# zfountas/deep-active-inference-mc

Measured on AMD Instinct MI355X. Metric: EFE rollouts/sec (64x64 dSprites, 10 MC-samples, depth 5), higher is better.
Workload: dtype f32; 1 GPU; calculate_G_repeated: 128 rows (32 roots x 4 actions) x depth 5 x 10 MC samples per GPU (BASELINE configs[1]) + action posterior; rows_per_gpu=128, samples=10, depth=5, parallelism=episodes sharded x1, weights replicated

## Files before the change

### deep-active-inference-mc_amd/csrc/decoder.hip

```cpp
#include <utility>
#include "mfma_pipe.h"

namespace efe {

template <class F, int... I> __device__ __forceinline__ void static_for_(F&& f, std::integer_sequence<int, I...>) { (f(std::integral_constant<int, I>{}), ...); }
template <int N, class F> __device__ __forceinline__ void static_for(F&& f) { static_for_(f, std::make_integer_sequence<int, N>{}); }

__host__ __device__ constexpr int w3_nch(int G) { return G == 4 ? 5 : 4; }
__host__ __device__ constexpr int w3_prod(int G, int c) {
    return G < 4 ? 5 * ((G >> 1) + 2 * (c >> 1)) + (G & 1) + 2 * (c & 1)
         : G == 4 ? (c < 2 ? 5 * (1 + 2 * c) + 4 : c < 4 ? 20 + 1 + 2 * (c - 2) : 24)
                  : (c < 2 ? 5 * (2 * c) + 4 : 20 + 2 * (c - 2));
}
__host__ __device__ constexpr bool w3_direct(int pp) { return f22_o1(pp / 5) < 0 && f22_o1(pp % 5) < 0; }
__host__ __device__ constexpr int w3_view(int pp) { return 3 * f22_view(pp / 5) + f22_view(pp % 5); }
__host__ __device__ constexpr int w3_mat(int pp) { return 4 * f22_wt(pp / 5) + f22_wt(pp % 5); }
__host__ __device__ constexpr bool w3_hits(int pp, int o) {
    const int r = o >> 2, c = o & 3, pr = pp / 5, pc = pp % 5;
    return (r == f22_o0(pr) || r == f22_o1(pr)) && (c == f22_o0(pc) || c == f22_o1(pc));
}
__host__ __device__ constexpr bool w3_seen(int G, int c, int o) {
    for (int g = 0; g < G; ++g)
        for (int k = 0; k < w3_nch(g); ++k) if (w3_hits(w3_prod(g, k), o)) return true;
    if (!w3_direct(w3_prod(G, c)))
        for (int k = 0; k < w3_nch(G); ++k)
            if ((w3_direct(w3_prod(G, k)) || k < c) && w3_hits(w3_prod(G, k), o)) return true;
    return false;
}
__host__ __device__ constexpr bool w3_uses_view(int G, int vi) {
    for (int k = 0; k < w3_nch(G); ++k) if (w3_view(w3_prod(G, k)) == vi) return true;
    return false;
}
__host__ __device__ constexpr bool f22_in(int a, int r) { return a == 0 ? r <= 1 : (a == 1 ? r == 1 : r >= 1); }
__host__ __device__ constexpr bool w3_reads(int G, int r, int c) {
    for (int vi = 0; vi < 9; ++vi) if (w3_uses_view(G, vi) && f22_in(vi / 3, r) && f22_in(vi % 3, c)) return true;
    return false;
}

constexpr int DA_PS = 17;
constexpr int DA_BIAS = 273 * DA_PS;

__host__ __device__ constexpr int wino_i0(int a) { return a == 0 ? 0 : (a == 2 ? 2 : 1); }
__host__ __device__ constexpr int wino_i1(int a) { return a == 0 ? 2 : (a == 1 ? 2 : (a == 2 ? 1 : 3)); }
__host__ __device__ constexpr float wino_s1(int a) { return a == 1 ? 1.0f : -1.0f; }
__host__ __device__ constexpr float wino_at(int r, int a) { return r == 0 ? (a < 3 ? 1.0f : 0.0f) : (a == 0 ? 0.0f : (a == 1 ? 1.0f : -1.0f)); }

template <int NR, int R0, class Pix>
__device__ __forceinline__ void wino_l1(f32x16 (&out)[NR][2], const float4* __restrict__ U, const float4* sm, const int h,
                                        const int mt_, Pix pix) {
    constexpr int PD = 4;
    const unsigned ln = (threadIdx.x & 63u) * 16u;
    const __amdgpu_buffer_rsrc_t ur = wrsrc(U);
    int mt = mt_; asm volatile("" : "+s"(mt));
    constexpr int a_lo = NR == 2 ? 0 : R0, a_hi = NR == 2 ? 4 : R0 + 3;
    auto ufrag = [&](int a, int b, int kc) { return wfrag(ur, ln, (size_t)(((4 * a + b) * 2 + mt) * 8 + kc) * 64); };
    auto bases = [&](int a, int b, int (&pb)[4]) {
        const int i0 = wino_i0(a), i1 = wino_i1(a), j0 = wino_i0(b), j1 = wino_i1(b);
        pb[0] = pix(i0, j0); pb[1] = pix(i0, j1); pb[2] = pix(i1, j0); pb[3] = pix(i1, j1);
    };
    float4 aq[PD], raw[4];
    int pb[4];
#pragma unroll
    for (int p = 0; p < PD; ++p) aq[p] = ufrag(a_lo, 0, p);
    bases(a_lo, 0, pb);
#pragma unroll
    for (int q = 0; q < 4; ++q) raw[q] = sm[pb[q] + h];
    f32x16 xacc;
    const f32x16 zero = {};
    auto otrans = [&](int a, int b, const f32x16& m, auto mask) {
        constexpr int MASK = decltype(mask)::value;
#pragma unroll
        for (int r = 0; r < NR; ++r) {
            if (!((MASK >> r) & 1)) continue;
            const float car = wino_at(R0 + r, a);
#pragma unroll
            for (int c = 0; c < 2; ++c) {
                const float cbc = wino_at(c, b);
                if (cbc == 0.0f) continue;
                const float cf = car * cbc;
#pragma unroll
                for (int e = 0; e < 16; ++e) out[r][c][e] = __builtin_fmaf(cf, m[e], out[r][c][e]);
            }
        }
    };
    auto xi_row = [&](int a, auto mask) {
        const float s1 = wino_s1(a);
        const int an = a + 1 < a_hi ? a + 1 : a;
#pragma unroll
        for (int b = 0; b < 4; ++b) {
            const float t1 = wino_s1(b);
#pragma unroll
            for (int kc = 0; kc < 8; ++kc) {
                const float4 av = aq[kc % PD];
                aq[kc % PD] = (b * 8 + kc + PD < 32) ? ufrag(a, (b * 8 + kc + PD) >> 3, (kc + PD) & 7) : ufrag(an, 0, (kc + PD) & 7);
                float4 v;
                {
                    const float4 c0 = make_float4(__builtin_fmaf(s1, raw[2].x, raw[0].x), __builtin_fmaf(s1, raw[2].y, raw[0].y),
                                                  __builtin_fmaf(s1, raw[2].z, raw[0].z), __builtin_fmaf(s1, raw[2].w, raw[0].w));
                    const float4 c1 = make_float4(__builtin_fmaf(s1, raw[3].x, raw[1].x), __builtin_fmaf(s1, raw[3].y, raw[1].y),
                                                  __builtin_fmaf(s1, raw[3].z, raw[1].z), __builtin_fmaf(s1, raw[3].w, raw[1].w));
                    v = make_float4(__builtin_fmaf(t1, c1.x, c0.x), __builtin_fmaf(t1, c1.y, c0.y), __builtin_fmaf(t1, c1.z, c0.z), __builtin_fmaf(t1, c1.w, c0.w));
                }
                if (kc < 7) {
#pragma unroll
                    for (int q = 0; q < 4; ++q) raw[q] = sm[pb[q] + 2 * (kc + 1) + h];
                } else {
                    if (b < 3) bases(a, b + 1, pb);
                    else bases(an, 0, pb);
#pragma unroll
                    for (int q = 0; q < 4; ++q) raw[q] = sm[pb[q] + h];
                }
                __builtin_amdgcn_sched_barrier(0);
                f32x16& x = xacc;
                x = __builtin_amdgcn_mfma_f32_32x32x2f32(av.x, v.x, kc == 0 ? zero : x, 0, 0, 0);
                x = __builtin_amdgcn_mfma_f32_32x32x2f32(av.y, v.y, x, 0, 0, 0);
                x = __builtin_amdgcn_mfma_f32_32x32x2f32(av.z, v.z, x, 0, 0, 0);
                x = __builtin_amdgcn_mfma_f32_32x32x2f32(av.w, v.w, x, 0, 0, 0);
            }
            otrans(a, b, xacc, mask);
        }
    };
    if constexpr (NR == 2) {
        xi_row(0, std::integral_constant<int, 1>{});
#pragma unroll 1
        for (int a = 1; a < 3; ++a) xi_row(a, std::integral_constant<int, 3>{});
        xi_row(3, std::integral_constant<int, 2>{});
    } else {
#pragma unroll 1
        for (int a = a_lo; a < a_hi; ++a) xi_row(a, std::integral_constant<int, 1>{});
    }
}
struct F22Nb { int xb, c2[3], r2; };
__device__ __forceinline__ f32x4 f22_wfrag(const __amdgpu_buffer_rsrc_t wr, const unsigned ln, int ct, int m, int kc) {
    return __builtin_bit_cast(f32x4, wfrag(wr, ln + (unsigned)kc * 1024u, (size_t)(m * 4 + ct) * 256));
}
constexpr int F22_PD = 2;
__device__ __forceinline__ void f22_l2_first(f32x4 (&aq)[F22_PD][5], const __amdgpu_buffer_rsrc_t wr, const int dn, const unsigned ln) {
    static_for<F22_PD>([&](auto p) {
        static_for<w3_nch(p >> 2)>([&](auto c) { aq[p][c] = f22_wfrag(wr, ln, dn, w3_mat(w3_prod(p >> 2, c)), p & 3); });
    });
}
__device__ __forceinline__ void f22_l2(f32x4 (&acc)[16], f32x4 (&aq)[F22_PD][5], const __amdgpu_buffer_rsrc_t wr, const int dn,
                                       const unsigned ln, const f32x4 bias4, const f32x4* smv, const F22Nb& nb) {
    constexpr int NST = 24;
    auto px = [&](int i, int jj, int kc) -> f32x4 {
        return smv[(jj == 2 ? nb.c2[i] : (i == 2 ? nb.r2 + jj * DA_PS : nb.xb + (16 * i + jj) * DA_PS)) + 4 * kc];
    };
    auto view = [&](const f32x4 (&x)[9], int vi) -> f32x4 {
        const int va = vi / 3, vb = vi % 3;
        auto cv = [&](int i) -> f32x4 { return vb == 0 ? x[3 * i] - x[3 * i + 1] : (vb == 1 ? x[3 * i + 1] : x[3 * i + 2] - x[3 * i + 1]); };
        return va == 0 ? cv(0) - cv(1) : (va == 1 ? cv(1) : cv(2) - cv(1));
    };
    const f32x4 zero4 = {};
    f32x4 tq[5], xr[9];
    static_for<9>([&](auto i) { if constexpr (w3_reads(0, i / 3, i % 3)) xr[i] = px(i / 3, i % 3, 0); });
    static_for<NST>([&](auto stc) {
        constexpr int ST = decltype(stc)::value, G = ST >> 2, KC = ST & 3, GN = (ST + 1) >> 2, KN = (ST + 1) & 3;
        constexpr int SP = (ST + F22_PD) % NST, GP = SP >> 2, KP = SP & 3;
        f32x4 vw[9], ac[5];
        static_for<9>([&](auto vi) { if constexpr (w3_uses_view(G, vi)) vw[vi] = view(xr, vi); });
#pragma unroll
        for (int c = 0; c < 5; ++c) ac[c] = aq[ST % F22_PD][c];
        static_for<w3_nch(GP)>([&](auto c) { aq[ST % F22_PD][c] = f22_wfrag(wr, ln, ST + F22_PD < NST ? 0 : dn, w3_mat(w3_prod(GP, c)), KP); });
        if constexpr (ST + 1 < NST)
            static_for<9>([&](auto i) { if constexpr (w3_reads(GN, i / 3, i % 3)) xr[i] = px(i / 3, i % 3, KN); });
        __builtin_amdgcn_sched_barrier(0);
#pragma unroll
        for (int e = 0; e < 4; ++e)
            static_for<w3_nch(G)>([&](auto c) {
                constexpr int PP = w3_prod(G, c);
                const float b = vw[w3_view(PP)][e], av = ac[c][e];
                if constexpr (w3_direct(PP)) {
                    constexpr int O = 4 * f22_o0(PP / 5) + f22_o0(PP % 5);
                    constexpr bool FIRST = KC == 0 && !w3_seen(G, c, O);
                    acc[O] = __builtin_amdgcn_mfma_f32_16x16x4f32(av, b, (FIRST && e == 0) ? bias4 : acc[O], 0, 0, 0);
                } else {
                    tq[c] = __builtin_amdgcn_mfma_f32_16x16x4f32(av, b, (KC == 0 && e == 0) ? zero4 : tq[c], 0, 0, 0);
                }
            });
        if constexpr (KC == 3)
            static_for<w3_nch(G)>([&](auto c) {
                constexpr int PP = w3_prod(G, c);
                if constexpr (!w3_direct(PP))
                    static_for<16>([&](auto o) {
                        if constexpr (w3_hits(PP, o)) {
                            if constexpr (w3_seen(G, c, o)) acc[o] = acc[o] + tq[c];
                            else acc[o] = bias4 + tq[c];
                        }
                    });
            });
    });
}
__device__ __forceinline__ void f22_l2_store(f32x4 (&acc)[16], const __amdgpu_buffer_rsrc_t yr, const unsigned yoff, const int ct, const bool on) {
#pragma unroll
    for (int orow = 0; orow < 4; ++orow)
#pragma unroll
        for (int c = 0; c < 2; ++c) {
            u32x4 lo, hi;
#pragma unroll
            for (int e = 0; e < 4; ++e) {
                const unsigned x0 = __builtin_bit_cast(unsigned, relu_bits(acc[4 * orow + c][e]));
                const unsigned x1 = __builtin_bit_cast(unsigned, relu_bits(acc[4 * orow + c + 2][e]));
                const auto sw = __builtin_amdgcn_permlane32_swap(x0, x1, false, false);
                lo[e] = sw[0]; hi[e] = sw[1];
            }
            const unsigned so = (unsigned)(((2 * (orow & 1) + c) * 4096 + 2 * ct * 512 + (orow >> 1) * 32) * 16);
            if (on) {
                __builtin_amdgcn_raw_buffer_store_b128(lo, yr, yoff, so, 0);
                __builtin_amdgcn_raw_buffer_store_b128(hi, yr, yoff, so + 512u * 16u, 0);
            }
        }
}

__global__ void __launch_bounds__(256, 2) k_dec_a(const DecAArgs a) {
    constexpr int NTHR = 256;
    constexpr int NPH = 2048 / NTHR;
    constexpr int NPE = 8;
    extern __shared__ __attribute__((aligned(16))) float4 sm[];
    const int tid = threadIdx.x;
    const int lane = tid & 63;
    const int w = __builtin_amdgcn_readfirstlane(tid >> 6);

    const float4* W1 = reinterpret_cast<const float4*>(a.w1);
    const float4* W2 = reinterpret_cast<const float4*>(a.w2);

    if ((int)blockIdx.x >= a.rows) return;
    int* const slot = reinterpret_cast<int*>(sm + DA_BIAS + 32);
    if (tid == 0) slot[0] = 2 * (int)gridDim.x + atomicAdd(a.queue, 1);
    int nimg = (int)blockIdx.x + (int)gridDim.x;
    f32x4 pf[2 * NPH];
    f32x4* smv = reinterpret_cast<f32x4*>(sm);
    {
        const f32x4* X = reinterpret_cast<const f32x4*>(a.x4) + (size_t)blockIdx.x * 4096;
#pragma unroll
        for (int it = 0; it < 2 * NPH; ++it) pf[it] = X[w * 1024 + it * 64 + lane];
    }
    for (int i = tid; i < 17 * DA_PS; i += NTHR) sm[256 * DA_PS + i] = make_float4(0.f, 0.f, 0.f, 0.f);
    if (tid < 16) sm[DA_BIAS + tid] = reinterpret_cast<const float4*>(a.b1)[tid];
    else if (tid < 32) sm[DA_BIAS + tid] = reinterpret_cast<const float4*>(a.b2)[tid - 16];

    for (int img = blockIdx.x; img < a.rows;) {
        int tl_ = tid; asm volatile("" : "+v"(tl_));
        const int j = tl_ & 31, h = (tl_ >> 5) & 1;
        const bool live = row_live(a.live, img);
        if (live) {
            const int sbase = (64 * w + ((tl_ >> 4) & 3)) * DA_PS + (tl_ & 15);
#pragma unroll
            for (int it = 0; it < 2 * NPH; ++it) smv[sbase + it * 4 * DA_PS] = pf[it];
        }
        __syncthreads();
        const int nnimg = slot[0];
        int ticket = 0;
        if (tid == 0) ticket = 2 * (int)gridDim.x + atomicAdd(a.queue, 1);
        const int l1mt = w >> 1, l1n = 32 * (w & 1) + j;
        const int l1y = 2 * (l1n >> 3) - 1, l1x = 2 * (l1n & 7) - 1;
        if (live) {
            f32x16 l1o[2][2];
#pragma unroll
            for (int g4 = 0; g4 < 4; ++g4) {
                const float4 bb = sm[DA_BIAS + l1mt * 8 + 2 * g4 + h];
#pragma unroll
                for (int rc = 0; rc < 4; ++rc) { l1o[rc >> 1][rc & 1][4 * g4] = bb.x; l1o[rc >> 1][rc & 1][4 * g4 + 1] = bb.y; l1o[rc >> 1][rc & 1][4 * g4 + 2] = bb.z; l1o[rc >> 1][rc & 1][4 * g4 + 3] = bb.w; }
            }
            wino_l1<2, 0>(l1o, W1, sm, h, l1mt, [&](int i, int jj) {
                const int y = l1y + i, x = l1x + jj;
                return ((unsigned)y < 16u && (unsigned)x < 16u ? y * 16 + x : 256) * DA_PS;
            });
            __syncthreads();
            if (tid == 0) slot[0] = ticket;
#pragma unroll
            for (int rc = 0; rc < 4; ++rc) {
                const int pix = (l1y + 1 + (rc >> 1)) * 16 + l1x + 1 + (rc & 1);
#pragma unroll
                for (int g4 = 0; g4 < 4; ++g4) {
                    const f32x16& o = l1o[rc >> 1][rc & 1];
                    float4 v;
                    v.x = relu_bits(o[4 * g4 + 0]); v.y = relu_bits(o[4 * g4 + 1]);
                    v.z = relu_bits(o[4 * g4 + 2]); v.w = relu_bits(o[4 * g4 + 3]);
                    sm[pix * DA_PS + l1mt * 8 + 2 * g4 + h] = v;
                }
            }
        } else {
            __syncthreads();
            if (tid == 0) slot[0] = ticket;
        }
        __syncthreads();
        {
            int t2_ = tid; asm volatile("" : "+v"(t2_));
            const int n = t2_ & 15, g = (t2_ >> 4) & 3;
            const int bu = 2 * w + (n >> 3), bv = n & 7;
            const int zq = 256 * DA_PS + g;
            F22Nb nb;
            nb.xb = (32 * bu + 2 * bv) * DA_PS + g;
            nb.c2[0] = bv == 7 ? zq : nb.xb + 2 * DA_PS;
            nb.c2[1] = bv == 7 ? zq : nb.xb + 18 * DA_PS;
            nb.c2[2] = bv == 7 ? zq : nb.xb + 34 * DA_PS;
            nb.r2 = nb.xb + 32 * DA_PS;
            const unsigned ln = (unsigned)(t2_ & 63) * 16u;
            const unsigned yoff = (unsigned)(((32 * bu + 2 * bv + (g >> 1)) * 2 + (g & 1)) * 16);
            const __amdgpu_buffer_rsrc_t yr = wrsrc(a.y2 + (size_t)__builtin_amdgcn_readfirstlane(img) * (32 * 32 * 64));
            auto load_next = [&](const int lo, const int hi) {
                const int pimg = __builtin_amdgcn_readfirstlane(nimg < a.rows ? nimg : img);
                const __amdgpu_buffer_rsrc_t xr = wrsrc(a.x4 + (size_t)pimg * 16384);
#pragma unroll
                for (int it = 0; it < 2 * NPH; ++it)
                    if (it >= lo && it < hi) pf[it] = __builtin_bit_cast(f32x4, wfrag(xr, (unsigned)(w * 16384 + (t2_ & 63) * 16 + (it & 3) * 1024), (size_t)(it >> 2) * 256));
            };
            if (live) {
                f32x4 aq[F22_PD][5], acc2[16];
                f22_l2_first(aq, wrsrc(W2), 0, ln);
                load_next(0, NPE);
#pragma unroll 1
                for (int ct = 0; ct < 4; ++ct) {
                    const f32x4 bias4 = smv[DA_BIAS + 16 + 4 * ct + g];
                    f22_l2(acc2, aq, wrsrc(W2 + ct * 256), ct < 3 ? 1 : 0, ln, bias4, smv, nb);
                    if (ct < 3) f22_l2_store(acc2, yr, yoff, ct, true);
                }
                load_next(NPE, 2 * NPH);
                f22_l2_store(acc2, yr, yoff, 3, true);
            } else {
                load_next(0, 2 * NPH);
            }
        }
        __syncthreads();
        img = nimg; nimg = nnimg;
    }
}

constexpr int DAS_IN = 6 * 16;
constexpr int DAS_L1 = 4 * 16;
constexpr int DAS_BIAS = (DAS_IN + 1 + DAS_L1 + 2) * DA_PS;
constexpr size_t DAS_LDS_BYTES = (DAS_BIAS + 32) * sizeof(float4);
__global__ void __launch_bounds__(256, 2) k_dec_a_s(const DecAArgs a) {
    extern __shared__ __attribute__((aligned(16))) float4 sm[];
    float4* sin = sm;
    float4* sl1 = sm + (DAS_IN + 1) * DA_PS;
    const int tid = threadIdx.x, lane = tid & 63;
    const int w = __builtin_amdgcn_readfirstlane(tid >> 6);
    const int j = lane & 31, h = lane >> 5;
    const int img = blockIdx.x >> 3, p = blockIdx.x & 7;
    if (!row_live(a.live, img)) return;
    const float4* W1 = reinterpret_cast<const float4*>(a.w1);
    const float4* W2 = reinterpret_cast<const float4*>(a.w2);
    {
        const float4* X = reinterpret_cast<const float4*>(a.x4) + (size_t)img * 4096;
        const int c4 = tid & 15, px0 = tid >> 4;
        float4 v[6];
#pragma unroll
        for (int it = 0; it < 6; ++it) {
            const int pix = px0 + 16 * it, lr = pix >> 4, y = 2 * p - 1 + lr;
            v[it] = (y >= 0 && y < 16) ? X[(y * 16 + (pix & 15)) * 16 + c4] : make_float4(0.f, 0.f, 0.f, 0.f);
        }
#pragma unroll
        for (int it = 0; it < 6; ++it) sin[(px0 + 16 * it) * DA_PS + c4] = v[it];
    }
    if (tid < 16) sin[DAS_IN * DA_PS + tid] = make_float4(0.f, 0.f, 0.f, 0.f);
    if (tid < 2 * DA_PS) sl1[DAS_L1 * DA_PS + tid] = make_float4(0.f, 0.f, 0.f, 0.f);
    if (tid < 16) sm[DAS_BIAS + tid] = reinterpret_cast<const float4*>(a.b1)[tid];
    else if (tid < 32) sm[DAS_BIAS + tid] = reinterpret_cast<const float4*>(a.b2)[tid - 16];
    __syncthreads();
    const int mt = w >> 1;
    {
        const int r = w & 1, n = j & 15;
        const int ly = 2 * (n >> 3) - 1, lx = 2 * (n & 7) - 1;
        f32x16 o[1][2];
#pragma unroll
        for (int g4 = 0; g4 < 4; ++g4) {
            const float4 bb = sm[DAS_BIAS + mt * 8 + 2 * g4 + h];
#pragma unroll
            for (int c = 0; c < 2; ++c) { o[0][c][4 * g4] = bb.x; o[0][c][4 * g4 + 1] = bb.y; o[0][c][4 * g4 + 2] = bb.z; o[0][c][4 * g4 + 3] = bb.w; }
        }
        auto pix = [&](int i, int jj) {
            const int sy = ly + 1 + i, x = lx + jj, y = 2 * p - 1 + sy;
            return ((unsigned)y < 16u && (unsigned)x < 16u ? sy * 16 + x : DAS_IN) * DA_PS;
        };
        if (r) wino_l1<1, 1>(o, W1, sin, h, mt, pix);
        else wino_l1<1, 0>(o, W1, sin, h, mt, pix);
        if (j < 16)
#pragma unroll
        for (int c = 0; c < 2; ++c)
#pragma unroll
            for (int g4 = 0; g4 < 4; ++g4) {
                float4 v;
                v.x = relu_bits(o[0][c][4 * g4 + 0]); v.y = relu_bits(o[0][c][4 * g4 + 1]);
                v.z = relu_bits(o[0][c][4 * g4 + 2]); v.w = relu_bits(o[0][c][4 * g4 + 3]);
                sl1[((ly + 1 + r) * 16 + lx + 1 + c) * DA_PS + mt * 8 + 2 * g4 + h] = v;
            }
    }
    __syncthreads();
    {
        const int n = lane & 15, g = lane >> 4, bv = n & 7;
        const int zq = DAS_L1 * DA_PS + g;
        F22Nb nb;
        nb.xb = 2 * bv * DA_PS + g;
        nb.c2[0] = bv == 7 ? zq : nb.xb + 2 * DA_PS;
        nb.c2[1] = bv == 7 ? zq : nb.xb + 18 * DA_PS;
        nb.c2[2] = (bv == 7 || p == 7) ? zq : nb.xb + 34 * DA_PS;
        nb.r2 = p == 7 ? zq : nb.xb + 32 * DA_PS;
        const unsigned ln = (unsigned)lane * 16u;
        const unsigned yoff = (unsigned)(((32 * p + 2 * bv + (g >> 1)) * 2 + (g & 1)) * 16);
        const __amdgpu_buffer_rsrc_t yr = wrsrc(a.y2 + (size_t)img * (32 * 32 * 64));
        const __amdgpu_buffer_rsrc_t wr = wrsrc(W2 + w * 256);
        f32x4 aq[F22_PD][5], acc2[16];
        f22_l2_first(aq, wr, 0, ln);
        const f32x4 bias4 = reinterpret_cast<const f32x4*>(sm)[DAS_BIAS + 16 + 4 * w + g];
        f22_l2(acc2, aq, wr, 0, ln, bias4, reinterpret_cast<const f32x4*>(sl1), nb);
        f22_l2_store(acc2, yr, yoff, w, n < 8);
    }
}

constexpr size_t DA_LDS_BYTES = (DA_BIAS + 33) * sizeof(float4);
int init_dec_b_kernels();
int init_decoder_kernels() {
    if (hipFuncSetAttribute((const void*)k_dec_a, hipFuncAttributeMaxDynamicSharedMemorySize, DA_LDS_BYTES) != hipSuccess) return 1;
    if (hipFuncSetAttribute((const void*)k_dec_a_s, hipFuncAttributeMaxDynamicSharedMemorySize, DAS_LDS_BYTES) != hipSuccess) return 1;
    return init_dec_b_kernels();
}

void launch_dec_a(const DecAArgs& a, hipStream_t st) {
    if (a.parts == 8) {
        hipLaunchKernelGGL(k_dec_a_s, dim3(a.rows * 8), dim3(256), DAS_LDS_BYTES, st, a);
        return;
    }
    const size_t lds = DA_LDS_BYTES;
    const int grid = a.rows < 512 ? a.rows : 512;
    hipLaunchKernelGGL(k_dec_a, dim3(grid), dim3(256), lds, st, a);
}


template <int PARTS>
__global__ void __launch_bounds__(256, 2) k_dec_b4(const DecBArgs a) {
    constexpr int SR = 4, NW = 4, NTHR = 256;
    constexpr int DB_RP = 33;
    constexpr int DB_PS = 17;
    constexpr int DB_IN_F4 = (SR + 1) * DB_RP * DB_PS;
    constexpr int DB_YROWS = 4 * SR + 2;
    constexpr int NPF = (SR + 1) * 512 / NTHR;
    constexpr int NS = 32 / SR;
    constexpr int NST = 24;
    extern __shared__ __attribute__((aligned(16))) float4 sm[];
    float* sH = reinterpret_cast<float*>(sm + DB_IN_F4);
    __shared__ float4 sb3[8];
    const int tid = threadIdx.x;
    const int lane = tid & 63;
    const int w = __builtin_amdgcn_readfirstlane(tid >> 6);
    const int g = lane >> 4, v = lane & 15;
    const int u = w >> 1, hf = w & 1;
    constexpr int parts = PARTS;
    const int img = parts == 1 ? (int)blockIdx.x : (int)(blockIdx.x >> 2);
    const int qtr = parts == 1 ? 0 : (int)(blockIdx.x & 3);
    if (!row_live(a.live, img)) return;
    const int s_lo = parts == 1 ? 0 : (qtr ? 2 * qtr - 1 : 0);
    const int s_hi = parts == 1 ? NS : 2 * qtr + 2;

    const int mg = a.m0 + img;
    const int gi = mg / a.rows_per_group;
    const int r = mg - gi * a.rows_per_group;
    int gt, gp, gs;
    group_decode(a.gm, gi, gt, gp, gs);
    const int mode = (gp == 0 && a.reward0) ? 1 : 0;
    const int slot = (gp == 0 && a.store0) ? gt * a.gm.S + gs : -1;
    float* po = (slot >= 0) ? a.po + ((size_t)slot * a.rows_per_group + r) * 4096 : nullptr;

    __shared__ float sq[4 * NTHR];
    __shared__ float sQ[4];
    if (tid < 8) sb3[tid] = reinterpret_cast<const float4*>(a.b3)[tid];
    if (tid < (SR + 1) * 16) sm[((tid >> 4) * DB_RP + 32) * DB_PS + (tid & 15)] = make_float4(0.f, 0.f, 0.f, 0.f);
    f32x4 w4a;
    {
        const int kh = v >> 2, kw = v & 3;
#pragma unroll
        for (int rr = 0; rr < 4; ++rr) w4a[rr] = (kh < 3 && kw < 3) ? a.w4[(3 * kh + kw) * 32 + 16 * hf + 4 * g + rr] : 0.f;
    }

    const __amdgpu_buffer_rsrc_t xr = __builtin_amdgcn_make_buffer_rsrc(const_cast<float*>(a.y2) + (size_t)img * (32 * 32 * 64), 0, 32 * 32 * 64 * 4, 0x00020000);
    const __amdgpu_buffer_rsrc_t wr = wrsrc(a.w3 + (size_t)hf * 4 * 64 * 4);
    const unsigned ln = (unsigned)lane * 16u;
    auto wf = [&](int m, int kc) -> f32x4 { return __builtin_bit_cast(f32x4, wfrag(wr, ln, (size_t)(m * 8 + kc) * 64)); };
    const float D1 = 1.00001f, D0 = 0.00001f;
    float part = 0.f;
    f32x4 pf[NPF];
    f32x4* smv = reinterpret_cast<f32x4*>(sm);
    auto prefetch = [&](int sn, int tl) {
        const unsigned lo = (unsigned)(((tl >> 5) * 512 + (tl & 31)) * 16);
        const unsigned lh = lo | (sn == NS - 1 ? 0x80000000u : 0u);
#pragma unroll
        for (int it = 0; it < NPF; ++it) {
            const int rl = it >> 1;
            const unsigned pc = (unsigned)((((rl & 1) * 16 + (it & 1) * 8) * 512 + (rl >> 1) * 32) * 16);
            pf[it] = __builtin_bit_cast(f32x4, __builtin_amdgcn_raw_buffer_load_b128(xr, rl == SR ? lh : lo, pc + (unsigned)sn * 1024u, 0));
        }
    };
    prefetch(s_lo, tid);

    const int xb = (2 * u * DB_RP + 2 * v) * DB_PS + g;
    auto px = [&](int i, int jj, int kc) -> f32x4 { return smv[xb + (i * DB_RP + jj) * DB_PS + 4 * kc]; };
    auto view = [&](const f32x4 (&x)[9], int vi) -> f32x4 {
        const int va = vi / 3, vb = vi % 3;
        auto cv = [&](int i) -> f32x4 { return vb == 0 ? sub4(x[3 * i], x[3 * i + 1]) : (vb == 1 ? x[3 * i + 1] : sub4(x[3 * i + 2], x[3 * i + 1])); };
        return va == 0 ? sub4(cv(0), cv(1)) : (va == 1 ? cv(1) : sub4(cv(2), cv(1)));
    };

    constexpr int RWG = 2 * SR / NW;
    float gh[RWG][6], gpr[RWG];
    auto g_load = [&](int oh, int q, int r0y, int hb0) {
#pragma unroll
        for (int kh = 0; kh < 3; ++kh) {
            const int tr = oh + 1 - kh;
            const bool rv = tr >= 0 && tr <= 63;
            int hs = hb0 + (tr - r0y);
            hs = hs < 0 ? hs + DB_YROWS : hs;
            hs = hs >= DB_YROWS ? hs - DB_YROWS : hs;
            hs = rv ? hs : 0;
            const float* hq = sH + ((hs * 2) * 3 + kh) * 64 + lane;
            gh[q][2 * kh] = hq[0]; gh[q][2 * kh + 1] = hq[3 * 64];
        }
    };
    auto g_sig = [&](int oh, int q) {
        float val = a.b4;
#pragma unroll
        for (int kh = 0; kh < 3; ++kh) {
            const int tr = oh + 1 - kh;
            val = add1(val, (tr >= 0 && tr <= 63) ? add1(gh[q][2 * kh], gh[q][2 * kh + 1]) : 0.f);
        }
        gpr[q] = hw_sigmoid(val);
    };
    auto g_term = [&](int oh, int q) {
#pragma clang fp contract(off)
        const float pr = gpr[q];
        const float l1 = hw_log(D1 - pr), l0 = hw_log(D0 + pr);
        const float te = __builtin_fmaf(pr - 1.0f, l1, -(pr * l0));
        const float tw = reward_term(pr, oh, lane, 64, 64, a.reward_intent);
        const float t = mode == 0 ? te : tw;
        part += oh >= 0 ? t : 0.0f;
    };
    auto g_store = [&](int oh, int q) {
        if (po && oh >= 0) {
            int owl = lane; asm volatile("" : "+v"(owl));
            (po + oh * 64)[owl] = gpr[q];
        }
    };

    auto fold = [&](int k) { sq[k * NTHR + tid] = part; part = 0.f; };
    float* const sHw = sH + g * 64 + 4 * v;
    int hb = 0, hbp = 0;
    for (int s = s_lo; s < s_hi; ++s) {
        int tl = tid; asm volatile("" : "+v"(tl));
        const bool gq = parts == 1 ? true : s == 2 * qtr + 1;
        const int oh0 = 2 * SR * (s - 1) - 1 + w, oh1 = oh0 + NW;
        {
            f32x4* const sp = smv + ((tl & 31) >> 1) * (2 * DB_PS) + 2 * (tl >> 5) + (tl & 1);
#pragma unroll
            for (int it = 0; it < NPF; ++it) sp[((it >> 1) * DB_RP + (it & 1)) * DB_PS] = pf[it];
        }
        f32x4 aq[5];
#pragma unroll
        for (int c = 0; c < w3_nch(0); ++c) aq[c] = wf(w3_mat(w3_prod(0, c)), 0);
        __syncthreads();

        const f32x4 bias4 = __builtin_bit_cast(f32x4, sb3[4 * hf + g]);
        const f32x4 zero4 = {};
        f32x4 acc[16], tq[5];
        f32x4 xr[9];
        static_for<9>([&](auto i) { if constexpr (w3_reads(0, i / 3, i % 3)) xr[i] = px(i / 3, i % 3, 0); });
        static_for<NST>([&](auto stc) {
            constexpr int ST = decltype(stc)::value, G = ST >> 2, KC = ST & 3, GN = (ST + 1) >> 2, KN = (ST + 1) & 3;
            f32x4 vw[9], ac[5];
            static_for<9>([&](auto vi) { if constexpr (w3_uses_view(G, vi)) vw[vi] = view(xr, vi); });
#pragma unroll
            for (int c = 0; c < 5; ++c) ac[c] = aq[c];
            if constexpr (ST + 1 < NST) {
                static_for<w3_nch(GN)>([&](auto c) { aq[c] = wf(w3_mat(w3_prod(GN, c)), KN); });
                static_for<9>([&](auto i) { if constexpr (w3_reads(GN, i / 3, i % 3)) xr[i] = px(i / 3, i % 3, KN); });
            }
            __builtin_amdgcn_sched_barrier(0);
#pragma unroll
            for (int e = 0; e < 4; ++e)
                static_for<w3_nch(G)>([&](auto c) {
                    constexpr int PP = w3_prod(G, c);
                    const float b = vw[w3_view(PP)][e], av = ac[c][e];
                    if constexpr (w3_direct(PP)) {
                        constexpr int O = 4 * f22_o0(PP / 5) + f22_o0(PP % 5);
                        constexpr bool FIRST = KC == 0 && !w3_seen(G, c, O);
                        acc[O] = __builtin_amdgcn_mfma_f32_16x16x4f32(av, b, (FIRST && e == 0) ? bias4 : acc[O], 0, 0, 0);
                    } else {
                        tq[c] = __builtin_amdgcn_mfma_f32_16x16x4f32(av, b, (KC == 0 && e == 0) ? zero4 : tq[c], 0, 0, 0);
                    }
                });
            if constexpr (KC == 3)
                static_for<w3_nch(G)>([&](auto c) {
                    constexpr int PP = w3_prod(G, c);
                    if constexpr (!w3_direct(PP))
                        static_for<16>([&](auto o) {
                            if constexpr (w3_hits(PP, o)) {
                                if constexpr (w3_seen(G, c, o)) acc[o] = add4(acc[o], tq[c]);
                                else acc[o] = add4(bias4, tq[c]);
                            }
                        });
                });
            if (gq) {
                if constexpr (ST == 0) { g_load(oh0, 0, 2 * SR * (s - 1), hbp); g_load(oh1, 1, 2 * SR * (s - 1), hbp); }
                if constexpr (ST == 2) g_sig(oh0, 0);
                if constexpr (ST == 5) g_term(oh0, 0);
                if constexpr (ST == 8) g_sig(oh1, 1);
                if constexpr (ST == 11) g_term(oh1, 1);
            }
        });
        prefetch((s < NS - 1) ? s + 1 : NS - 1, tl);
#pragma unroll
        for (int orow = 0; orow < 4; ++orow) {
            f32x4 T[4];
#pragma unroll
            for (int oc = 0; oc < 4; ++oc)
#pragma unroll
                for (int e = 0; e < 4; ++e) acc[4 * orow + oc][e] = relu_bits(acc[4 * orow + oc][e]);
#pragma unroll
            for (int e = 0; e < 4; ++e)
#pragma unroll
                for (int oc = 0; oc < 4; ++oc)
                    T[oc] = __builtin_amdgcn_mfma_f32_16x16x4f32(w4a[e], acc[4 * orow + oc][e], e == 0 ? zero4 : T[oc], 0, 0, 0);
            f32x4 hv;
            hv[0] = add1(add1(T[1][0], T[0][1]), dpp_shr1_zero(T[3][2]));
            hv[1] = add1(add1(T[2][0], T[1][1]), T[0][2]);
            hv[2] = add1(add1(T[3][0], T[2][1]), T[1][2]);
            hv[3] = add1(add1(dpp_shl1_zero(T[0][0]), T[3][1]), T[2][2]);
            int hsw = hb + 4 * u + orow;
            hsw = hsw >= DB_YROWS ? hsw - DB_YROWS : hsw;
            if (g < 3) *reinterpret_cast<f32x4*>(sHw + (hsw * 2 + hf) * (3 * 64)) = hv;
        }
        __syncthreads();
        if (gq) { g_store(oh0, 0); g_store(oh1, 1); }
        if (parts == 1 && (s == 2 || s == 4 || s == 6)) fold(s / 2 - 1);
        if (s == s_hi - 1) {
#pragma unroll
            for (int q = 0; q <= RWG; ++q) {
                if (q == RWG && (w != 0 || s != NS - 1)) break;
                const int oh = 2 * SR * s - 1 + q * NW + w;
                g_load(oh, 0, 2 * SR * s, hb); g_sig(oh, 0); g_term(oh, 0); g_store(oh, 0);
            }
        }
        hbp = hb;
        hb += 2 * SR;
        hb = hb >= DB_YROWS ? hb - DB_YROWS : hb;
    }
    fold(parts == 1 ? 3 : 0);
    __syncthreads();
    if (w < (parts == 1 ? 4 : 1)) {
        const float* qk = sq + w * NTHR + lane;
        float val = add1(add1(qk[0], qk[64]), add1(qk[128], qk[192]));
#pragma unroll
        for (int o = 32; o > 0; o >>= 1) val += __shfl_xor(val, o);
        if (lane == 0) sQ[w] = val;
    }
    __syncthreads();
    if (tid == 0) {
        if (parts == 1) a.val[mg] = add1(add1(sQ[0], sQ[1]), add1(sQ[2], sQ[3]));
        else a.valq[(size_t)mg * 4 + qtr] = sQ[0];
    }
}

constexpr size_t DB_LDS4D = ((5 * 33) * 17) * sizeof(float4) + 18 * 2 * 3 * 64 * sizeof(float);
int init_dec_b_kernels() {
    if (hipFuncSetAttribute((const void*)k_dec_b4<1>, hipFuncAttributeMaxDynamicSharedMemorySize, DB_LDS4D) != hipSuccess) return 1;
    if (hipFuncSetAttribute((const void*)k_dec_b4<4>, hipFuncAttributeMaxDynamicSharedMemorySize, DB_LDS4D) != hipSuccess) return 1;
    return 0;
}

void launch_dec_b(const DecBArgs& a, hipStream_t st) {
    if (a.parts == 4) hipLaunchKernelGGL(k_dec_b4<4>, dim3(a.rows * 4), dim3(256), DB_LDS4D, st, a);
    else hipLaunchKernelGGL(k_dec_b4<1>, dim3(a.rows), dim3(256), DB_LDS4D, st, a);
}

__host__ __device__ inline int fc4_spg(int mtiles) { return ((mtiles + 7) / 8 + 7) / 8; }
template <int NT>
__global__ void __launch_bounds__(256, 2) k_fc4(const GemmArgs a) {
    constexpr int RT = 32 * NT;
    extern __shared__ __attribute__((aligned(16))) float4 sm[];
    const int tid = threadIdx.x;
    const int lane = tid & 63;
    const int w = __builtin_amdgcn_readfirstlane(tid >> 6);
    const int j = lane & 31, h = lane >> 5;
    const int fgrp = blockIdx.x & 7;
    const int nper = gridDim.x >> 3, k = blockIdx.x >> 3;
    const int SPG = fc4_spg(a.mtiles);
    const int nsteps = ((a.n_pix + RT - 1) / RT) * SPG;
    const int q0 = (int)(((long)nsteps * k) / nper), q1 = (int)(((long)nsteps * (k + 1)) / nper);
    f32x4* smv = reinterpret_cast<f32x4*>(sm);
    const float4* Wl = reinterpret_cast<const float4*>(a.Wp);
    auto xaddr = [&](int t, int (&bs)[NT], int (&sw)[NT], int& wt) {
        wt = t;
#pragma unroll
        for (int nt = 0; nt < NT; ++nt) { bs[nt] = (nt * 32 + j) * 64 + t * 16; sw[nt] = j & 15; }
    };
    int cur_rt = -1;
    uint32_t krow[2] = {0, 0}, kstream[2] = {0, 0}, kstage[2] = {0, 0};
    bool rv[2] = {false, false};
#pragma unroll 1
    for (int q = q0; q < q1; ++q) {
        const int rt = q / SPG, fs = q - rt * SPG;
        const int row0 = rt * RT;
        if (rt != cur_rt) {
            if (cur_rt >= 0) __syncthreads();
            cur_rt = rt;
            const f32x4* X = reinterpret_cast<const f32x4*>(a.X);
#pragma unroll
            for (int it = 0; it < 8 * NT; ++it) {
                const int idx = it * 256 + tid;
                const int r = idx >> 6, c4 = idx & 63;
                const int gr = row0 + r;
                smv[r * 64 + (c4 ^ (r & 15))] = (gr < a.n_pix) ? X[(size_t)gr * 64 + c4] : (f32x4)(0.f);
            }
            __syncthreads();
#pragma unroll
            for (int nt = 0; nt < NT; ++nt) {
                const int m = row0 + nt * 32 + j;
                rv[nt] = m < a.n_pix;
                const int mg = a.m0 + (rv[nt] ? m : 0);
                const int g = mg / a.rows_per_group;
                krow[nt] = global_row(a.gm.ids, a.gm.ids_div, mg - g * a.rows_per_group, a.row_offset);
                const uint2 key = group_key(a.gm, g);
                kstream[nt] = key.x; kstage[nt] = key.y;
            }
        }
        const int mt0 = (fgrp * SPG + fs) * 8 + 2 * w;
        if (mt0 >= a.mtiles) continue;
        f32x16 acc[2][NT];
#pragma unroll
        for (int mt = 0; mt < 2; ++mt)
#pragma unroll
            for (int nt = 0; nt < NT; ++nt)
#pragma unroll
                for (int e = 0; e < 16; ++e) acc[mt][nt][e] = 0.f;
        float4 bq[2][4];
#pragma unroll
        for (int mt = 0; mt < 2; ++mt)
#pragma unroll
            for (int g4 = 0; g4 < 4; ++g4) bq[mt][g4] = *reinterpret_cast<const float4*>(a.bias + (mt0 + mt) * 32 + 8 * g4 + 4 * h);
        tap_loop<2, NT>(acc, 4, Wl, sm, h, xaddr, DenseWIdx{mt0});
#pragma unroll
        for (int nt = 0; nt < NT; ++nt) {
            if (!rv[nt]) continue;
            const uint4 rnd = noise_words(a.k0, a.k1, a.tag, (uint32_t)((mt0 * 32) >> 7), krow[nt], kstream[nt], kstage[nt]);
            float* yp = a.Y + (size_t)(row0 + nt * 32 + j) * a.ldy;
#pragma unroll
            for (int mt = 0; mt < 2; ++mt)
#pragma unroll
                for (int g4 = 0; g4 < 4; ++g4) {
                    const int co = (mt0 + mt) * 32 + 8 * g4 + 4 * h;
                    const float4 bb = bq[mt][g4];
                    const uint32_t word = ((co >> 5) & 3) == 0 ? rnd.x : ((co >> 5) & 3) == 1 ? rnd.y : ((co >> 5) & 3) == 2 ? rnd.z : rnd.w;
                    float v[4] = {acc[mt][nt][4 * g4 + 0] + bb.x, acc[mt][nt][4 * g4 + 1] + bb.y,
                                  acc[mt][nt][4 * g4 + 2] + bb.z, acc[mt][nt][4 * g4 + 3] + bb.w};
#pragma unroll
                    for (int e = 0; e < 4; ++e) v[e] = ((word >> ((co + e) & 31)) & 1u) ? fmaxf(v[e], 0.f) * 2.0f : 0.0f;
                    *reinterpret_cast<float4*>(yp + co) = make_float4(v[0], v[1], v[2], v[3]);
                }
        }
    }
}

void launch_fc4(const GemmArgs& a, hipStream_t st) {
    if (a.n_pix <= 32) {
        const int nsteps = fc4_spg(a.mtiles);
        hipLaunchKernelGGL(k_fc4<1>, dim3(8 * (nsteps < 64 ? nsteps : 64)), dim3(256), 32 * 64 * sizeof(float4), st, a);
        return;
    }
    const int nsteps = ((a.n_pix + 63) / 64) * fc4_spg(a.mtiles);
    const int nper = nsteps < 64 ? nsteps : 64;
    hipLaunchKernelGGL(k_fc4<2>, dim3(8 * nper), dim3(256), 64 * 64 * sizeof(float4), st, a);
}

}
```

Before: 11800 rollouts/s.

## Interleave four Winograd columns with independent MFMA accumulators in wino_l1

Restructures the Winograd layer-1 loop so all four b-columns of a row are processed together per k-chunk. Each column gets its own accumulator, so MFMA chains are interleaved instead of serially dependent. The input-side transform is shared: eight raw pixels are loaded once per k-chunk and combined into four column vectors, replacing repeated per-column loads. This removes MFMA dependency stalls and redundant LDS reads, at the cost of more registers (four f32x16 accumulators plus eight raw float4s), which may reduce occupancy or cause spills.

```diff
diff --git a/deep-active-inference-mc_amd/csrc/decoder.hip b/deep-active-inference-mc_amd/csrc/decoder.hip
--- a/deep-active-inference-mc_amd/csrc/decoder.hip
+++ b/deep-active-inference-mc_amd/csrc/decoder.hip
@@ -48,24 +48,24 @@
 template <int NR, int R0, class Pix>
 __device__ __forceinline__ void wino_l1(f32x16 (&out)[NR][2], const float4* __restrict__ U, const float4* sm, const int h,
                                         const int mt_, Pix pix) {
-    constexpr int PD = 4;
     const unsigned ln = (threadIdx.x & 63u) * 16u;
     const __amdgpu_buffer_rsrc_t ur = wrsrc(U);
     int mt = mt_; asm volatile("" : "+s"(mt));
     constexpr int a_lo = NR == 2 ? 0 : R0, a_hi = NR == 2 ? 4 : R0 + 3;
     auto ufrag = [&](int a, int b, int kc) { return wfrag(ur, ln, (size_t)(((4 * a + b) * 2 + mt) * 8 + kc) * 64); };
-    auto bases = [&](int a, int b, int (&pb)[4]) {
-        const int i0 = wino_i0(a), i1 = wino_i1(a), j0 = wino_i0(b), j1 = wino_i1(b);
-        pb[0] = pix(i0, j0); pb[1] = pix(i0, j1); pb[2] = pix(i1, j0); pb[3] = pix(i1, j1);
-    };
-    float4 aq[PD], raw[4];
-    int pb[4];
-#pragma unroll
-    for (int p = 0; p < PD; ++p) aq[p] = ufrag(a_lo, 0, p);
-    bases(a_lo, 0, pb);
-#pragma unroll
-    for (int q = 0; q < 4; ++q) raw[q] = sm[pb[q] + h];
-    f32x16 xacc;
+    auto bases = [&](int a, int (&pb)[8]) {
+        const int i0 = wino_i0(a), i1 = wino_i1(a);
+#pragma unroll
+        for (int jj = 0; jj < 4; ++jj) { pb[jj] = pix(i0, jj); pb[4 + jj] = pix(i1, jj); }
+    };
+    float4 aq[4], raw[8];
+    int pb[8];
+#pragma unroll
+    for (int b = 0; b < 4; ++b) aq[b] = ufrag(a_lo, b, 0);
+    bases(a_lo, pb);
+#pragma unroll
+    for (int q = 0; q < 8; ++q) raw[q] = sm[pb[q] + h];
+    f32x16 xacc[4];
     const f32x16 zero = {};
     auto otrans = [&](int a, int b, const f32x16& m, auto mask) {
         constexpr int MASK = decltype(mask)::value;
@@ -87,38 +87,41 @@
         const float s1 = wino_s1(a);
         const int an = a + 1 < a_hi ? a + 1 : a;
 #pragma unroll
-        for (int b = 0; b < 4; ++b) {
-            const float t1 = wino_s1(b);
-#pragma unroll
-            for (int kc = 0; kc < 8; ++kc) {
-                const float4 av = aq[kc % PD];
-                aq[kc % PD] = (b * 8 + kc + PD < 32) ? ufrag(a, (b * 8 + kc + PD) >> 3, (kc + PD) & 7) : ufrag(an, 0, (kc + PD) & 7);
-                float4 v;
-                {
-                    const float4 c0 = make_float4(__builtin_fmaf(s1, raw[2].x, raw[0].x), __builtin_fmaf(s1, raw[2].y, raw[0].y),
-                                                  __builtin_fmaf(s1, raw[2].z, raw[0].z), __builtin_fmaf(s1, raw[2].w, raw[0].w));
-                    const float4 c1 = make_float4(__builtin_fmaf(s1, raw[3].x, raw[1].x), __builtin_fmaf(s1, raw[3].y, raw[1].y),
-                                                  __builtin_fmaf(s1, raw[3].z, raw[1].z), __builtin_fmaf(s1, raw[3].w, raw[1].w));
-                    v = make_float4(__builtin_fmaf(t1, c1.x, c0.x), __builtin_fmaf(t1, c1.y, c0.y), __builtin_fmaf(t1, c1.z, c0.z), __builtin_fmaf(t1, c1.w, c0.w));
+        for (int kc = 0; kc < 8; ++kc) {
+            float4 av[4], v[4];
+#pragma unroll
+            for (int b = 0; b < 4; ++b) {
+                av[b] = aq[b];
+                aq[b] = kc < 7 ? ufrag(a, b, kc + 1) : ufrag(an, b, 0);
+            }
+            {
+                float4 c[4];
+#pragma unroll
+                for (int jj = 0; jj < 4; ++jj)
+                    c[jj] = make_float4(__builtin_fmaf(s1, raw[4 + jj].x, raw[jj].x), __builtin_fmaf(s1, raw[4 + jj].y, raw[jj].y),
+                                        __builtin_fmaf(s1, raw[4 + jj].z, raw[jj].z), __builtin_fmaf(s1, raw[4 + jj].w, raw[jj].w));
+#pragma unroll
+                for (int b = 0; b < 4; ++b) {
+                    const float t1 = wino_s1(b);
+                    const float4 c0 = c[wino_i0(b)], c1 = c[wino_i1(b)];
+                    v[b] = make_float4(__builtin_fmaf(t1, c1.x, c0.x), __builtin_fmaf(t1, c1.y, c0.y), __builtin_fmaf(t1, c1.z, c0.z), __builtin_fmaf(t1, c1.w, c0.w));
                 }
-                if (kc < 7) {
-#pragma unroll
-                    for (int q = 0; q < 4; ++q) raw[q] = sm[pb[q] + 2 * (kc + 1) + h];
-                } else {
-                    if (b < 3) bases(a, b + 1, pb);
-                    else bases(an, 0, pb);
-#pragma unroll
-                    for (int q = 0; q < 4; ++q) raw[q] = sm[pb[q] + h];
-                }
-                __builtin_amdgcn_sched_barrier(0);
-                f32x16& x = xacc;
-                x = __builtin_amdgcn_mfma_f32_32x32x2f32(av.x, v.x, kc == 0 ? zero : x, 0, 0, 0);
-                x = __builtin_amdgcn_mfma_f32_32x32x2f32(av.y, v.y, x, 0, 0, 0);
-                x = __builtin_amdgcn_mfma_f32_32x32x2f32(av.z, v.z, x, 0, 0, 0);
-                x = __builtin_amdgcn_mfma_f32_32x32x2f32(av.w, v.w, x, 0, 0, 0);
-            }
-            otrans(a, b, xacc, mask);
-        }
+            }
+            if (kc == 7) bases(an, pb);
+#pragma unroll
+            for (int q = 0; q < 8; ++q) raw[q] = sm[pb[q] + (kc < 7 ? 2 * (kc + 1) : 0) + h];
+            __builtin_amdgcn_sched_barrier(0);
+#pragma unroll
+            for (int b = 0; b < 4; ++b) xacc[b] = __builtin_amdgcn_mfma_f32_32x32x2f32(av[b].x, v[b].x, kc == 0 ? zero : xacc[b], 0, 0, 0);
+#pragma unroll
+            for (int b = 0; b < 4; ++b) xacc[b] = __builtin_amdgcn_mfma_f32_32x32x2f32(av[b].y, v[b].y, xacc[b], 0, 0, 0);
+#pragma unroll
+            for (int b = 0; b < 4; ++b) xacc[b] = __builtin_amdgcn_mfma_f32_32x32x2f32(av[b].z, v[b].z, xacc[b], 0, 0, 0);
+#pragma unroll
+            for (int b = 0; b < 4; ++b) xacc[b] = __builtin_amdgcn_mfma_f32_32x32x2f32(av[b].w, v[b].w, xacc[b], 0, 0, 0);
+        }
+#pragma unroll
+        for (int b = 0; b < 4; ++b) otrans(a, b, xacc[b], mask);
     };
     if constexpr (NR == 2) {
         xi_row(0, std::integral_constant<int, 1>{});
```

New measurement: 11880 rollouts/s (median of 6 runs). Within noise of the previous version (+0.7%).
